# Sudaraka88/LDWeaver

Measured on AMD Instinct MI355X. Metric: MI SNP-pairs/sec, higher is better.
Workload: dtype i8

## Files before the change

include/ldweaver_amd_debug.h:

```cpp
#ifndef LDWEAVER_AMD_DEBUG_H
#define LDWEAVER_AMD_DEBUG_H

#include "ldweaver_amd.h"

#ifdef __cplusplus
extern "C" {
#endif

#define LDW_ENGINE_MFMA 0
#define LDW_ENGINE_HIST 1
#define LDW_ENGINE_HIST_STATES 2

int ldw_build_info(void);
int ldw_ctx_last_timing(ldw_ctx *ctx, double ms_out[4]);
int ldw_ctx_counters(ldw_ctx *ctx, int64_t out[4]);
int ldw_ctx_counters2(ldw_ctx *ctx, int64_t out[8]);
int ldw_gemm_stats(ldw_ctx *ctx, double out[6], int reset);
int ldw_apx_info(ldw_ctx *ctx, double out[6]);

int ldw_hamming_stats(ldw_ctx *ctx, double out[8]);
int ldw_joint_tables(ldw_ctx *ctx, const int32_t *pair_a, const int32_t *pair_b, int64_t npairs,
                     int64_t *counts_out, int64_t *fixed_out, int *frac_bits_out);

int ldw_set_engine(ldw_ctx *ctx, int engine);
int ldw_set_overlap(ldw_ctx *ctx, int on);
int ldw_set_fused(ldw_ctx *ctx, int on);
int ldw_set_mixed(ldw_ctx *ctx, int on);
int ldw_set_path(ldw_ctx *ctx, int mode);
int ldw_set_select(ldw_ctx *ctx, int mode);
int ldw_set_screen(ldw_ctx *ctx, int mode);
int ldw_set_prune(ldw_ctx *ctx, int on);
int ldw_set_pair_cap(uint32_t cap);
int ldw_reset_speculation(ldw_ctx *ctx);

int ldw_path_report(ldw_ctx *ctx, int64_t out[8], char *gate, int capacity);
int ldw_pair_form_report(ldw_ctx *ctx, int64_t out[5]);
int ldw_prune_report(ldw_ctx *ctx, int64_t out[4]);
int ldw_span_report(ldw_ctx *ctx, int64_t out[4]);
int ldw_overflow_report(ldw_ctx *ctx, int64_t out[4]);

int ldw_snp_bounds(ldw_ctx *ctx, double *out, int64_t capacity);
int ldw_debug_violations(ldw_ctx *ctx, double *out);
int ldw_debug_tab11(ldw_ctx *ctx, double W, double lo, double delta, double eta, double sprime, int32_t *out, double *cbin_out);
int ldw_debug_apx_params(ldw_ctx *ctx, double out[20], int64_t *vfixed_out, int64_t *vapx_out, int64_t capacity);
int ldw_debug_rows(ldw_ctx *ctx, int32_t *row0_out, uint32_t *slot_meta_out, int64_t capacity);
int ldw_debug_apx_gemm(ldw_ctx *ctx, const int32_t *rows_t, int nrt, const int32_t *rows_f, int nrf, int32_t *out);
int ldw_debug_screen_bound(ldw_ctx *ctx, int kind, int na, int nb, int64_t n, const int64_t *g, const int64_t *pa, const int64_t *pb, const float *pX, const float *pY,
                           const double *rr, const uint32_t *masks, const double params[20], float *out, double *out64);

int ldw_debug_plot_panels(ldw_ctx *ctx, const double *x, const double *y, const double *srp, const uint8_t *layer, const uint8_t *panel, int64_t n,
                          int on_device, const ldw_plot_opts *opts, int n_panels, int32_t W, int32_t H, uint8_t *rgb_out, double *stats_out,
                          int64_t *scratch_bytes_out, double *ms_out);
int ldw_debug_plot_colours(int kind, const double *t, int64_t n, uint8_t *rgb_out);
int ldw_tsv_stats(ldw_ctx *ctx, double *out10);
int ldw_tsv_set_variant(ldw_ctx *ctx, int variant);

#ifdef __cplusplus
}
#endif
#endif
```

ldweaver_amd/_lib.py:

```python
from __future__ import annotations

import ctypes as C
import os

import numpy as np

_HERE = os.path.dirname(os.path.abspath(__file__))
LIB_PATH = os.environ.get("LDW_AMD_LIB") or os.path.join(_HERE, "libldweaver_amd.so")

LDW_OK = 0
LDW_ERR_ARG, LDW_ERR_HIP, LDW_ERR_STATE, LDW_ERR_NOGPU, LDW_ERR_SIZE = 1, 2, 3, 4, 5
QUIRK_REFERENCE, QUIRK_INTENDED = 0, 1
MI_SR_ROWS_STAY = 1
ENGINE_MFMA, ENGINE_HIST, ENGINE_HIST_STATES = 0, 1, 2
COL_INT32, COL_INT64, COL_DOUBLE, COL_STR = 0, 1, 2, 3


class LdwError(RuntimeError):
    def __init__(self, code: int, msg: str):
        super().__init__(f"libldweaver_amd error {code}: {msg}")
        self.code = code


PLOT_SR_CLUST, PLOT_SR_COMBI, PLOT_LR, PLOT_LDMAP = 0, 1, 2, 3
# ... 99 lines not shown
    "ldw_write_alignment": (C.c_int, [_p, C.c_char_p, C.c_int, C.c_int, _p, _i64, C.c_char_p, _i64, _i64, C.POINTER(_i64)]),
    "ldw_write_table_tsv_str": (C.c_int, [C.c_char_p, C.c_int, _i64, C.c_int, _p, _p, _p, _p, _p, _i64, C.c_int, C.POINTER(_i64)]),
    "ldw_annot_snps": (C.c_int, [_p, _p, _i64, _p, _i64, _p, _i64, _p, _p, _i64, _p]),
    "ldw_annot_map": (C.c_int, [_p, _p, _p, _i64, _p, _i64, _p, C.POINTER(_i64), C.POINTER(_i64)]),
    "ldw_annot_links": (C.c_int, [_p, _p, _p, _i64, _p, _p, _i64, _i64, _p, _p, _p, _p, _p, C.POINTER(_i64)]),
    "ldw_plot_layout_get": (C.c_int, [C.c_int, C.c_int, C.c_double, C.c_double, C.c_double, C.c_double, _p]),
    "ldw_plot_ticks": (C.c_int, [C.c_double, C.c_double, C.c_int, C.c_int, _p, _p, _p, _p]),
    "ldw_png_write": (C.c_int, [C.c_char_p, _p, C.c_int32, C.c_int32, C.c_int, C.POINTER(_i64)]),
    "ldw_plot_scatter": (C.c_int, [_p, _p, _p, _p, _p, _p, _i64, C.c_int, _p, C.c_int, _p, C.c_char_p, _p, C.POINTER(_i64)]),
    "ldw_plot_links": (C.c_int, [_p, C.c_int, C.c_int, _p, C.c_char_p, _p, C.POINTER(_i64)]),
    "ldw_plot_heatmap": (C.c_int, [_p, _p, C.c_int32, C.c_int, C.c_char_p, C.c_char_p, _p]),
    "ldw_plot_ldmap": (C.c_int, [_p, C.c_int32, C.c_int32, C.c_int32, C.c_char_p, C.c_char_p, _p, _p, _p, _p, _i64]),
    "ldw_tsv_probe": (C.c_int, [C.c_char_p, C.c_int, C.POINTER(C.c_int32), C.POINTER(C.c_int32)]),
    "ldw_tsv_read": (C.c_int, [_p, C.c_char_p, C.c_int, C.c_int32, _i64, C.POINTER(_i64), C.POINTER(_i64), C.POINTER(C.c_uint32)]),
    "ldw_tsv_columns": (C.c_int, [_p, C.POINTER(_p), C.POINTER(_i64), C.POINTER(C.c_int32), C.POINTER(_i64)]),
    "ldw_tsv_fetch": (C.c_int, [_p, C.c_int32, _p, _i64, C.c_int]),
    "ldw_set_positions": (C.c_int, [_p, _p, _i64, C.c_double]),
    "ldw_links_load": (C.c_int, [_p, C.c_int, C.c_int32, C.c_int32, C.c_int32, C.c_int32, C.c_double, C.c_int32, C.POINTER(_i64)]),
    "ldw_compare_to_row": (C.c_int, [_p, _i64, _i64, _p, _i64, _p]),
    "ldw_vec_pos_match": (C.c_int, [_p, _i64, _p, _i64, _p]),
    "ldw_compare_triplet": (C.c_int, [_p, _p, _i64, C.c_double, C.POINTER(C.c_int)]),
    "ldw_fast_intersect": (C.c_int, [_p, _i64, _p, _i64, _p, C.POINTER(_i64)]),
}
_SIGS_DEBUG = {
    "ldw_build_info": (C.c_int, []),
    "ldw_ctx_last_timing": (C.c_int, [_p, _p]),
    "ldw_ctx_counters": (C.c_int, [_p, _p]),
    "ldw_ctx_counters2": (C.c_int, [_p, _p]),
    "ldw_gemm_stats": (C.c_int, [_p, _p, C.c_int]),
    "ldw_apx_info": (C.c_int, [_p, _p]),
    "ldw_hamming_stats": (C.c_int, [_p, _p]),
    "ldw_joint_tables": (C.c_int, [_p, _p, _p, _i64, _p, _p, _p]),
    "ldw_set_engine": (C.c_int, [_p, C.c_int]),
    "ldw_set_overlap": (C.c_int, [_p, C.c_int]),
    "ldw_set_fused": (C.c_int, [_p, C.c_int]),
    "ldw_set_mixed": (C.c_int, [_p, C.c_int]),
    "ldw_set_path": (C.c_int, [_p, C.c_int]),
    "ldw_set_select": (C.c_int, [_p, C.c_int]),
    "ldw_set_screen": (C.c_int, [_p, C.c_int]),
    "ldw_set_prune": (C.c_int, [_p, C.c_int]),
    "ldw_set_pair_cap": (C.c_int, [C.c_uint32]),
    "ldw_reset_speculation": (C.c_int, [_p]),
    "ldw_path_report": (C.c_int, [_p, _p, C.c_char_p, C.c_int]),
    "ldw_pair_form_report": (C.c_int, [_p, _p]),
    "ldw_prune_report": (C.c_int, [_p, _p]),
    "ldw_span_report": (C.c_int, [_p, _p]),
    "ldw_overflow_report": (C.c_int, [_p, _p]),
    "ldw_snp_bounds": (C.c_int, [_p, _p, C.c_int64]),
    "ldw_debug_violations": (C.c_int, [_p, _p]),
    "ldw_debug_tab11": (C.c_int, [_p, C.c_double, C.c_double, C.c_double, C.c_double, C.c_double, _p, _p]),
    "ldw_debug_apx_params": (C.c_int, [_p, _p, _p, _p, _i64]),
    "ldw_debug_rows": (C.c_int, [_p, _p, _p, _i64]),
    "ldw_debug_apx_gemm": (C.c_int, [_p, _p, C.c_int, _p, C.c_int, _p]),
    "ldw_debug_screen_bound": (C.c_int, [_p, C.c_int, C.c_int, C.c_int, _i64, _p, _p, _p, _p, _p, _p, _p, _p, _p, _p]),
    "ldw_debug_plot_panels": (C.c_int, [_p, _p, _p, _p, _p, _p, _i64, C.c_int, _p, C.c_int, C.c_int32, C.c_int32, _p, _p, C.POINTER(_i64), _p]),
    "ldw_debug_plot_colours": (C.c_int, [C.c_int, _p, _i64, _p]),
    "ldw_tsv_stats": (C.c_int, [_p, _p]),
    "ldw_tsv_set_variant": (C.c_int, [_p, C.c_int]),
}
_SIGS = {**_SIGS_API, **_SIGS_DEBUG}
_SIGS_BY_HEADER = {"ldweaver_amd.h": _SIGS_API, "ldweaver_amd_debug.h": _SIGS_DEBUG}


def declared_symbols(header: str | None = None):
    return sorted(_SIGS if header is None else _SIGS_BY_HEADER[header])


def lib():
    global _lib
    if _lib is None:
        if not os.path.exists(LIB_PATH):
            raise FileNotFoundError(
                f"{LIB_PATH} not found: build it with `make -C ldweaver_amd/csrc` or "
                "`python -c 'import __graft_entry__ as g; g.build()'` — there is no CPU fallback")
        try:
            import torch
        except ImportError:
            pass
        l = C.CDLL(LIB_PATH)
        for name, (res, args) in _SIGS.items():
            fn = getattr(l, name)
            fn.restype = res
            fn.argtypes = args
        _lib = l
    return _lib


def has_experiments() -> bool:
    return bool(lib().ldw_build_info() & 1)


def check(code: int):
    if code != LDW_OK:
        raise LdwError(code, lib().ldw_last_error().decode("utf-8", "replace"))


def ptr(a):
    if a is None:
        return None
    if isinstance(a, int):
        return C.c_void_p(a)
    if isinstance(a, np.ndarray):
        return C.c_void_p(a.ctypes.data)
    if hasattr(a, "data_ptr"):
        return C.c_void_p(a.data_ptr())
    raise TypeError(f"cannot take a pointer of {type(a)}")
# ... 6 lines not shown
```

ldweaver_amd/csrc/ldw_api.hip:

```cpp
#include <algorithm>
#include <atomic>
#include <chrono>
#include <cmath>
#include <cstdarg>
#include <cstdio>
#include <cstdlib>
#include <cstring>

#include <thread>
#include "ldw_internal.h"
#include "ldw_dev.h"
#include "ldw_fasta.h"
#include "ldw_links_read.h"

namespace ldw {
static thread_local char g_err[1024] = "";

void set_error(const char *fmt, ...) {
    va_list ap;
    va_start(ap, fmt);
    vsnprintf(g_err, sizeof(g_err), fmt, ap);
    va_end(ap);
}

// ... 384 lines not shown

int launch_fasta_count_pack(const uint8_t *chunk, int64_t rows, int64_t L, int64_t Lp, int32_t *counts, uint8_t *packed, hipStream_t s) {
    const int64_t lanes = (L + FA_COLS - 1) / FA_COLS;
    hipLaunchKernelGGL(k_fasta_count_pack, dim3((unsigned)((lanes + 255) / 256)), dim3(256), 0, s, chunk, rows, L, Lp, counts, packed);
    LDW_HIP(hipGetLastError());
    return LDW_OK;
}

int launch_fasta_encode_rows(bool packed, const uint8_t *src, int64_t stride, int64_t src_s0, int64_t s0, int64_t s_end, int64_t N,
                             const int32_t *pos, int64_t n_pos, uint8_t *states, int64_t Npad, hipStream_t s) {
    const dim3 grid((unsigned)((n_pos + 63) / 64), (unsigned)((s_end - s0 + 63) / 64));
    if (packed)
        hipLaunchKernelGGL(k_fasta_encode_rows<true>, grid, dim3(256), 0, s, src, stride, src_s0, s0, s_end, N, pos, n_pos, states, Npad);
    else
        hipLaunchKernelGGL(k_fasta_encode_rows<false>, grid, dim3(256), 0, s, src, stride, src_s0, s0, s_end, N, pos, n_pos, states, Npad);
    LDW_HIP(hipGetLastError());
    return LDW_OK;
}

}

extern "C" {

int ldw_version(void) { return 100; }

const char *ldw_last_error(void) { return ldw::g_err; }

int ldw_build_info(void) { return 0; }

int ldw_device_count(void) {
    int n = 0;
    if (hipGetDeviceCount(&n) != hipSuccess) return 0;
    return n;
}

int ldw_ctx_create(int device, ldw_ctx **out) {
    LDW_REQUIRE(out != nullptr, LDW_ERR_ARG, "ldw_ctx_create: out is null");
    int n = 0;
    if (hipGetDeviceCount(&n) != hipSuccess || n <= 0) {
        set_error("ldw_ctx_create: no HIP device visible; this library has no CPU fallback");
        return LDW_ERR_NOGPU;
    }
    LDW_REQUIRE(device >= 0 && device < n, LDW_ERR_ARG, "ldw_ctx_create: device %d out of range (0..%d)", device, n - 1);
    LDW_HIP(hipSetDevice(device));
    hipDeviceProp_t prop;
    LDW_HIP(hipGetDeviceProperties(&prop, device));
    if (strncmp(prop.gcnArchName, "gfx950", 6) != 0) {
        set_error("ldw_ctx_create: device %d is %s; kernels are built for gfx950 only", device, prop.gcnArchName);
        return LDW_ERR_NOGPU;
    }
    ldw_ctx *c = new ldw_ctx();
    ldw::ctx_count(+1);
    c->device = device;
    c->prune = getenv("LDW_NO_PRUNE") == nullptr;
    LDW_HIP(hipStreamCreateWithFlags(&c->stream, hipStreamNonBlocking));
    c->own_stream = true;
    for (auto &e : c->ev) LDW_HIP(hipEventCreate(&e));
    static const bool no_prep = getenv("LDW_NO_PREPARE") != nullptr;
    if (!no_prep) {
        if (int rc = ldw::ensure_streams(c)) {
            const std::string msg = ldw_last_error();
            ldw_ctx_destroy(c);
            *out = nullptr;
            ldw::set_error("%s", msg.c_str());
            return rc;
        }
        c->prep_thread = new std::thread([c] {
            int rc = LDW_OK;
            if (hipSetDevice(c->device) != hipSuccess) rc = LDW_ERR_HIP;
            if (rc == LDW_OK) {
                ldw::warm_mi();
                ldw::warm_apx();
                ldw::warm_gemm_bits();
                ldw::warm_srp();
                ldw::warm_post();
            }
            if (rc != LDW_OK) c->prep_err = ldw_last_error();
            c->prep_rc = rc;
        });
    }
    *out = c;
    return LDW_OK;
}

int ldw_ctx_reserve(ldw_ctx *c, int64_t L, int64_t N, int64_t max_blk_sz) {
    if (int rc = check_gpu(c)) return rc;
    LDW_REQUIRE(L > 0 && N > 0 && max_blk_sz > 0, LDW_ERR_ARG, "ldw_ctx_reserve: L, N and max_blk_sz must be positive");
    if (c->prep_thread2) {
        if (c->prep_thread2->joinable()) c->prep_thread2->join();
        delete c->prep_thread2;
        c->prep_thread2 = nullptr;
    }
    static const bool no_prep = getenv("LDW_NO_PREPARE") != nullptr;
    if (no_prep) return LDW_OK;
    const int64_t blk = std::min<int64_t>(L, max_blk_sz);
    const int64_t nblk = (L + blk - 1) / blk;
    const int64_t nseg = std::max<int64_t>(1, std::min<int64_t>(c->span_on ? c->span_max : 1, nblk - 2));
    const int64_t nt = blk * nseg, rows_f = blk * 5 / 4 + 512, rows_t = nt * 5 / 4 + 512;
    const size_t stage = (size_t)((blk + nt) * 12 + (rows_f + rows_t) * 9 + nt * 52 + (blk + 64) * 16 + 3 * (rows_t / 128 + 1) * (rows_f / 64 + 1) + 65536);
    const int64_t Npad = (N + ldw::KSTEP - 1) / ldw::KSTEP * ldw::KSTEP;
    c->prep_thread2 = new std::thread([c, stage, Npad, blk, nseg] {
        int rc = LDW_OK;
        if (hipSetDevice(c->device) != hipSuccess) rc = LDW_ERR_HIP;
        if (rc == LDW_OK) rc = ldw::reserve_slot_buffers(c, Npad, blk, nseg);
        for (int k = 0; k < LDW_NSLOT && rc == LDW_OK; ++k) {
            if (c->pin_cap[k] >= stage) continue;
// ... 767 lines not shown
```

ldweaver_amd/csrc/ldw_apx.hip:

```cpp
#include <algorithm>
#include <cmath>
#include <cstdlib>
#include <cstring>

#include "ldw_apx.h"
#include "ldw_dev.h"

using namespace ldw;

namespace ldw {

namespace {
constexpr int64_t APX_PROD_CAP = 12000;
struct ProdTable {
    std::vector<int32_t> val;
    std::vector<uint8_t> a, b;
    ProdTable() {
        std::vector<std::pair<int32_t, std::pair<uint8_t, uint8_t>>> all;
        for (int x = 0; x <= 127; ++x)
            for (int y = x; y <= 127; ++y) all.push_back({x * y, {(uint8_t)x, (uint8_t)y}});
        std::sort(all.begin(), all.end());
        for (auto &e : all)
            if (val.empty() || val.back() != e.first) {
                val.push_back(e.first);
// ... 321 lines not shown
        if (valid && !(P.sr_mask && P.sr_mask[(int64_t)((ty * TH) / 128) * (P.RFpad / 64) + tx] != 0)) {
            const TileSummary F = apx_fold_rows(P.bin_f + (int64_t)tx * TWd, P.rflag_f ? P.rflag_f + (int64_t)tx * TWd : nullptr, TWd);
            all_binned = T.bmax < P.tab_nb && F.bmax < P.tab_nb;
            if (P.rflag_t) {
                const unsigned kt = T.fand & PF_KIND, kf = F.fand & PF_KIND;
                pruned = kt >= 2u && kt == (T.forr & PF_KIND) && kf >= 2u && kf == (F.forr & PF_KIND) &&
                         ((T.fand & (kf == 2u ? PF_DEAD2 : PF_DEAD3)) != 0u || (F.fand & (kt == 2u ? PF_DEAD2 : PF_DEAD3)) != 0u);
            }
            if (!pruned && all_binned && (T.bmax - T.bmin + 1) * (F.bmax - F.bmin + 1) <= 64) {
                bool ok = true;
                for (int bt = T.bmin; bt <= T.bmax; ++bt)
                    for (int bf = F.bmin; bf <= F.bmax; ++bf) {
                        const int2 th = P.tab[bt * P.tab_nb + bf];
                        ok = ok && th.x < 0 && th.y == 2147483647;
                    }
                pruned = ok;
            }
        }
        if (pruned && all_binned) {
#pragma unroll
            for (int i = 0; i < MT; ++i)
#pragma unroll
                for (int h = 0; h < (NT * 32) / 64; ++h) P.clean[(int64_t)((ty * TH + 32 * i) / 32) * (P.RFpad / 64) + (tx * TWd) / 64 + h] = 1;
        }
        const bool live = valid && !pruned;
        const unsigned long long lm = __ballot(live);
        n_pruned += (unsigned int)__popcll(__ballot(valid && pruned));
        if (lane == 0) s_wave[wave] = (unsigned int)__popcll(lm);
        __syncthreads();
        if (threadIdx.x == 0) {
            const unsigned int tot = s_wave[0] + s_wave[1] + s_wave[2] + s_wave[3];
            s_base = tot ? atomicAdd(P.n_live, tot) : 0u;
        }
        __syncthreads();
        unsigned int off = s_base;
        for (int w = 0; w < wave; ++w) off += s_wave[w];
        if (live) P.tile_list[off + (unsigned int)__popcll(lm & ((1ull << lane) - 1ull))] = (uint32_t)(ty * ntx + tx);
        __syncthreads();
    }
    if (lane == 0 && n_pruned) atomicAdd(P.skip_ctr, (unsigned long long)n_pruned);
}

template <int MT, int NT, bool FINE, int WPS = 2>
__global__ __launch_bounds__(256, WPS) void gemm_apx_kernel(ApxGemmArgs P) {
    extern __shared__ __attribute__((aligned(16))) uint8_t smem[];
    uint64_t *lutFF = reinterpret_cast<uint64_t *>(smem);
    uint8_t *sA = smem + APX_LUT_BYTES, *sB = sA + (size_t)P.M2 * 128;
    int2 *s_tab = reinterpret_cast<int2 *>(sB + (size_t)P.M2 * 128);
    const int tid = threadIdx.x;
    const int lane = tid & 63, wave = tid >> 6;
    constexpr int TH = 32 * MT, TWd = 32 * NT;
    int ty = 2 * blockIdx.y + (wave >> 1), tx = 2 * blockIdx.x + (wave & 1);
    bool outside;
    if (P.tile_list) {
        const unsigned int n_live = *P.n_live;
        if (blockIdx.x * 4u >= n_live) return;
        const unsigned int k = blockIdx.x * 4u + (unsigned int)wave;
        outside = k >= n_live;
        const int t = outside ? 0 : (int)P.tile_list[k];
        const int ntx = P.RFpad / TWd;
        ty = t / ntx;
        tx = t - ty * ntx;
    } else {
        outside = ty * TH >= P.RTpad || tx * TWd >= P.RFpad || (P.lower_only && tx * TWd + TWd - 1 < ty * TH);
    }
    if (P.fuse)
        for (int i = tid; i < P.tab_nb * P.tab_nb; i += 256) s_tab[i] = P.tab[i];
    {
        uint64_t e = 0;
#pragma unroll
        for (int k = 0; k < 8; ++k) e |= ((tid >> k) & 1) ? (0xFFull << (8 * k)) : 0ull;
        lutFF[tid] = e;
        const int n16 = P.M2 * 8;
        for (int i = tid; i < n16; i += 256) {
            reinterpret_cast<uint4 *>(sA)[i] = reinterpret_cast<const uint4 *>(P.dig_a)[i];
            reinterpret_cast<uint4 *>(sB)[i] = reinterpret_cast<const uint4 *>(P.dig_b)[i];
        }
    }
    __syncthreads();
    if (outside) return;
    const int frow = lane & 31, fh = lane >> 5;
    const int64_t sta = (int64_t)P.RTpad * 2, stb = (int64_t)P.RFpad * 2;
    {
        const apx_u32x4 *pa[MT], *pb[NT];
#pragma unroll
        for (int i = 0; i < MT; ++i) {
            const int rt = ty * TH + 32 * i + frow;
            pa[i] = reinterpret_cast<const apx_u32x4 *>(P.panel_t) + ((int64_t)rt * 2 + fh);
        }
#pragma unroll
        for (int i = 0; i < NT; ++i) {
            const int rf = tx * TWd + 32 * i + frow;
            pb[i] = reinterpret_cast<const apx_u32x4 *>(P.panel_f) + ((int64_t)rf * 2 + fh);
        }
        v16i acc[MT][NT];
#pragma unroll
        for (int i = 0; i < MT; ++i)
#pragma unroll
            for (int j = 0; j < NT; ++j)
#pragma unroll
                for (int e = 0; e < 16; ++e) acc[i][j][e] = 0;
        apx_u32x4 wa[MT], wb[NT], na[MT], nb[NT];
        const uint8_t *lut_bytes = smem;
#pragma unroll
        for (int i = 0; i < MT; ++i) na[i] = pa[i][0];
#pragma unroll
        for (int i = 0; i < NT; ++i) nb[i] = pb[i][0];
        for (int m = 0; m < P.M2; ++m) {
#pragma unroll
            for (int i = 0; i < MT; ++i) wa[i] = na[i];
#pragma unroll
            for (int i = 0; i < NT; ++i) wb[i] = nb[i];
            if (m + 1 < P.M2) {
#pragma unroll
                for (int i = 0; i < MT; ++i) na[i] = pa[i][(int64_t)(m + 1) * sta];
#pragma unroll
                for (int i = 0; i < NT; ++i) nb[i] = pb[i][(int64_t)(m + 1) * stb];
            }
            const int4 sh4 = reinterpret_cast<const int4 *>(P.shift)[m];
            const int shk[4] = {sh4.x, sh4.y, sh4.z, sh4.w};
            const uint8_t *dA = sA + m * 128 + fh * (FINE ? 16 : 64), *dB = sB + m * 128 + fh * (FINE ? 16 : 64);
            auto kstep = [&](auto KKc) {
                constexpr int kk = decltype(KKc)::value;
                const int sh = shk[kk];
                if ((FINE || kk == 0) && sh) {
#pragma unroll
                    for (int i = 0; i < MT; ++i)
#pragma unroll
                        for (int j = 0; j < NT; ++j)
#pragma unroll
                            for (int e = 0; e < 16; ++e) acc[i][j][e] = (int)((unsigned)acc[i][j][e] >> sh);
                }
                const v4i da = *reinterpret_cast<const v4i *>(dA + (FINE ? 32 : 16) * kk);
                const v4i db = *reinterpret_cast<const v4i *>(dB + (FINE ? 32 : 16) * kk);
                v4i fa[MT], fb[NT];
#pragma unroll
                for (int i = 0; i < MT; ++i) fa[i] = expand16s<kk>(lut_bytes, wa[i]) & da;
#pragma unroll
                for (int i = 0; i < NT; ++i) fb[i] = expand16s<kk>(lut_bytes, wb[i]) & db;
#pragma unroll
                for (int i = 0; i < MT; ++i)
#pragma unroll
                    for (int j = 0; j < NT; ++j) acc[i][j] = __builtin_amdgcn_mfma_i32_32x32x32_i8(fa[i], fb[j], acc[i][j], 0, 0, 0);
            };
            kstep(std::integral_constant<int, 0>{});
            kstep(std::integral_constant<int, 1>{});
            kstep(std::integral_constant<int, 2>{});
            kstep(std::integral_constant<int, 3>{});
        }
        apx_gemm_epilogue<MT, NT>(P, acc, ty, tx, lane, s_tab, reinterpret_cast<uint8_t *>(s_tab + 64 * 64) + wave * 256);
    }
}

int launch_apx_live_tiles(ldw_ctx *c, const ApxGemmArgs &P, hipStream_t st) {
    LDW_REQUIRE(P.fuse && P.skip_ctr && P.tile_list && P.n_live && P.RTpad % 128 == 0 && P.RFpad % 64 == 0 && P.tab && P.tab_nb == 64,
                LDW_ERR_ARG, "launch_apx_live_tiles: bad pruning arguments");
    hipLaunchKernelGGL(k_apx_live_tiles, dim3((unsigned)(P.RTpad / (32 * APX_MT))), dim3(256), 0, st, P);
    LDW_HIP(hipGetLastError());
    return LDW_OK;
}

int launch_gemm_apx(ldw_ctx *c, const ApxGemmArgs &P, hipStream_t st) {
    LDW_REQUIRE(P.RTpad % APX_TW == 0 && P.RFpad % APX_TW == 0 && P.M2 > 0, LDW_ERR_ARG, "launch_gemm_apx: padding violated (RT %d RF %d M2 %d)", P.RTpad,
                P.RFpad, P.M2);
    const size_t lds = APX_LUT_BYTES + (size_t)P.M2 * 256 + (P.fuse ? (size_t)P.tab_nb * P.tab_nb * 8 + 1024 : 0);
    LDW_REQUIRE(lds <= 65536, LDW_ERR_ARG, "launch_gemm_apx: %d positions do not fit the LDS digit arrays", P.M2 * 128);
    LDW_REQUIRE(!P.fuse || (P.tab_nb == 64 && P.bin_t && P.bin_f && P.tab && P.clean), LDW_ERR_ARG, "launch_gemm_apx: bad table arguments");
    if (P.skip_ctr) {
        LDW_REQUIRE(P.fuse && P.tile_list && P.n_live && P.RFpad % 64 == 0, LDW_ERR_ARG, "launch_gemm_apx: bad pruning arguments");
        const int tiles = (P.RTpad / (32 * APX_MT)) * (P.RFpad / 64), g = (tiles + 3) / 4;
        if (P.fine) hipLaunchKernelGGL((gemm_apx_kernel<APX_MT, 2, true, APX_WPS>), dim3((unsigned)g), dim3(256), lds, st, P);
        else hipLaunchKernelGGL((gemm_apx_kernel<APX_MT, 2, false, APX_WPS>), dim3((unsigned)g), dim3(256), lds, st, P);
    } else {
        const int ntx = P.RFpad / 64, nty = P.RTpad / 128;
        const dim3 grid((unsigned)((ntx + 1) / 2), (unsigned)((nty + 1) / 2));
        if (P.fine) hipLaunchKernelGGL((gemm_apx_kernel<4, 2, true>), grid, dim3(256), lds, st, P);
        else hipLaunchKernelGGL((gemm_apx_kernel<4, 2, false>), grid, dim3(256), lds, st, P);
    }
    LDW_HIP(hipGetLastError());
    {
        constexpr int TH = 128, TWd = 64;
        int64_t waves = 0;
        for (int ty = 0; ty * TH < P.RTpad; ++ty) {
            const int ntx = P.RFpad / TWd;
            if (!P.lower_only) waves += ntx;
            else for (int tx = 0; tx < ntx; ++tx) waves += (tx * TWd + TWd - 1 < ty * TH) ? 0 : 1;
        }
        c->gemm_stat[0] += 1;
        if (P.fuse) c->gemm_stat[5] += 1;
        c->gemm_stat[1] += 2.0 * (double)waves * TH * TWd * ((double)P.M2 * 128.0);
        if (P.fuse && P.skip_ctr) {
            c->apx_ops_per_wave = 2.0 * TH * TWd * ((double)P.M2 * 128.0);
            c->apx_waves_total += waves;
        }
    }
    return LDW_OK;
}

struct PairArgs {
    const uint64_t *Mbits;
    int64_t KW;
    int nwords, path, nseg;
    int seg_in_lds;
    const PopSeg *segs;
    const int32_t *wbeg, *row0;
    int32_t zero_row;
    int64_t *sums;
    EpiArgs A;
    unsigned long long *ghist;
};

template <int CA, int CB>
__device__ __forceinline__ void pair_sums_body(const PairArgs &P, int path, const int32_t *s_wbeg, const PopSeg *s_segs) {
    constexpr bool GENB = CA == 4 && CB == 4;
    const EpiArgs &A = P.A;
    const int sub = path * PAIR_SHARDS + (int)blockIdx.y;
    unsigned int n = A.pl_n[sub];
    n = n > A.pl_cap ? A.pl_cap : n;
    const int lane = threadIdx.x & 63;
    const PairEnt *list = A.pl_pairs + (int64_t)sub * A.pl_cap;
    constexpr int KW = 3, KS = 2;
    uint32_t smask[KW][KS];
    int64_t sV[KW][KS];
// ... 363 lines not shown
```

ldweaver_amd/csrc/ldw_debug.hip:

```cpp
#include <algorithm>
#include <cmath>
#include <cstring>
#include <vector>

#include "ldw_apx.h"
#include "ldw_dev.h"

using namespace ldw;

namespace ldw {

struct DbgArrays {
    const int64_t *g;
    const int32_t *g32;
    const int64_t *pa, *pb;
    const float *pX, *pY;
    const double *rr;
    const uint32_t *mk;
    float *out;
    double *out64;
    int64_t n;
};

template <int NA, int NB>
// ... 118 lines not shown
    if (int rc = check_gpu(c)) return rc;
    if (int rc = ensure_rows(c)) return rc;
    LDW_REQUIRE(row0_out && slot_meta_out && capacity >= c->L + 1, LDW_ERR_ARG, "ldw_debug_rows: need L + 1 = %lld entries", (long long)c->L + 1);
    memcpy(row0_out, c->h_row0.data(), (size_t)(c->L + 1) * 4);
    memcpy(slot_meta_out, c->h_slot_meta.data(), (size_t)c->L * 4);
    return LDW_OK;
}

int ldw_debug_apx_gemm(ldw_ctx *c, const int32_t *rows_t, int nrt, const int32_t *rows_f, int nrf, int32_t *out) {
    if (int rc = check_gpu(c)) return rc;
    if (int rc = join_prepare(c)) return rc;
    if (int rc = ensure_rows(c)) return rc;
    LDW_REQUIRE(rows_t && rows_f && out && nrt > 0 && nrf > 0 && nrt <= 8192 && nrf <= 8192, LDW_ERR_ARG, "ldw_debug_apx_gemm: bad argument");
    LDW_REQUIRE(c->apx_ok, LDW_ERR_STATE, "ldw_debug_apx_gemm: the weights do not allow the approximate path (%s)", c->apx_gate.c_str());
    for (int k = 0; k < nrt; ++k) LDW_REQUIRE(rows_t[k] >= 0 && rows_t[k] <= c->R, LDW_ERR_ARG, "ldw_debug_apx_gemm: to-side row %d = %d outside 0..R", k, rows_t[k]);
    for (int k = 0; k < nrf; ++k) LDW_REQUIRE(rows_f[k] >= 0 && rows_f[k] <= c->R, LDW_ERR_ARG, "ldw_debug_apx_gemm: from-side row %d = %d outside 0..R", k, rows_f[k]);
    const int RTpad = (nrt + APX_TW - 1) / APX_TW * APX_TW, RFpad = (nrf + APX_TW - 1) / APX_TW * APX_TW, M2 = (int)(c->KW / 2);
    std::vector<int32_t> rl((size_t)RTpad + RFpad, (int32_t)c->R);
    std::copy(rows_t, rows_t + nrt, rl.begin());
    std::copy(rows_f, rows_f + nrf, rl.begin() + RTpad);
    DevBuf d_rl, d_pt, d_pf, d_G;
    int rc = LDW_OK;
    if ((rc = d_rl.reserve(rl.size() * 4)) || (rc = d_pt.reserve((size_t)M2 * RTpad * 32)) || (rc = d_pf.reserve((size_t)M2 * RFpad * 32)) ||
        (rc = d_G.reserve((size_t)RTpad * RFpad * 4))) {
        d_rl.release(); d_pt.release(); d_pf.release(); d_G.release();
        return rc;
    }
    auto body = [&]() -> int {
        LDW_HIP(hipMemcpyAsync(d_rl.p, rl.data(), rl.size() * 4, hipMemcpyHostToDevice, c->stream));
        LDW_HIP(hipMemsetAsync(d_G.p, 0xFF, (size_t)RTpad * RFpad * 4, c->stream));
        if (int r2 = launch_pack_panel(c, d_rl.as<int32_t>() + RTpad, RFpad, d_pf.as<uint64_t>(), c->stream, d_rl.as<int32_t>(), RTpad, d_pt.as<uint64_t>())) return r2;
        ApxGemmArgs P;
        memset(&P, 0, sizeof(P));
        P.panel_t = d_pt.as<uint64_t>();
        P.panel_f = d_pf.as<uint64_t>();
        P.RTpad = RTpad;
        P.RFpad = RFpad;
        P.M2 = M2;
        P.dig_a = c->dig_a.as<uint8_t>();
        P.dig_b = c->dig_b.as<uint8_t>();
        P.shift = c->apx_shift.as<int32_t>();
        P.G = d_G.as<int32_t>();
        P.fine = c->apx_fine ? 1 : 0;
        if (int r2 = launch_gemm_apx(c, P, c->stream)) return r2;
        std::vector<int32_t> h((size_t)RTpad * RFpad);
        LDW_HIP(hipMemcpyAsync(h.data(), d_G.p, h.size() * 4, hipMemcpyDeviceToHost, c->stream));
        LDW_HIP(hipStreamSynchronize(c->stream));
        for (int t = 0; t < nrt; ++t) memcpy(out + (size_t)t * nrf, h.data() + (size_t)t * RFpad, (size_t)nrf * 4);
        return LDW_OK;
    };
    rc = body();
    (void)hipStreamSynchronize(c->stream);
    d_rl.release(); d_pt.release(); d_pf.release(); d_G.release();
    return rc;
}

int ldw_debug_screen_bound(ldw_ctx *c, int kind, int na, int nb, int64_t n, const int64_t *g, const int64_t *pa, const int64_t *pb, const float *pX, const float *pY,
                           const double *rr, const uint32_t *masks, const double params[20], float *out, double *out64) {
    if (int rc = check_gpu(c)) return rc;
    LDW_REQUIRE(n > 0 && n < ((int64_t)1 << 28) && g && pa && pb && pX && pY && rr && params, LDW_ERR_ARG, "ldw_debug_screen_bound: bad argument");
    LDW_REQUIRE(kind >= 0 && kind <= 4 && ((kind == 4) ? out64 != nullptr : out != nullptr), LDW_ERR_ARG, "ldw_debug_screen_bound: kind %d / missing output", kind);
    const bool generic = kind == 1 || kind == 3;
    LDW_REQUIRE(generic ? masks != nullptr : ((na == 1 || na == 2) && (nb == 1 || nb == 2)), LDW_ERR_ARG, "ldw_debug_screen_bound: kinds 0 / 2 / 4 take na, nb in {1, 2}; kinds 1 / 3 take masks");
    const bool apx = kind == 0 || kind == 1;
    std::vector<int32_t> g32;
    if (apx) {
        g32.resize((size_t)n * 16);
        for (size_t k = 0; k < g32.size(); ++k) {
            LDW_REQUIRE(g[k] >= -2147483647LL && g[k] <= 2147483647LL, LDW_ERR_ARG, "ldw_debug_screen_bound: entry %zu does not fit int32", k);
            g32[k] = (int32_t)g[k];
        }
    }
    DevBuf B;
    const size_t sz_g = (size_t)n * 16 * 8, sz_g32 = (size_t)n * 16 * 4, sz_p = (size_t)n * 5 * 8, sz_f = (size_t)n * 5 * 4, sz_r = (size_t)n * 3 * 8, sz_m = (size_t)n * 2 * 4,
                 sz_o = (size_t)n * 4, sz_o64 = (size_t)n * 8;
    auto al = [](size_t x) { return (x + 255) / 256 * 256; };
    const size_t o_g = 0, o_g32 = o_g + al(sz_g), o_pa = o_g32 + al(sz_g32), o_pb = o_pa + al(sz_p), o_pX = o_pb + al(sz_p), o_pY = o_pX + al(sz_f), o_rr = o_pY + al(sz_f),
                 o_m = o_rr + al(sz_r), o_o = o_m + al(sz_m), o_o64 = o_o + al(sz_o), total = o_o64 + al(sz_o64);
    if (int rc = B.reserve(total)) return rc;
    char *base = B.as<char>();
    auto body = [&]() -> int {
        LDW_HIP(hipMemcpyAsync(base + o_g, g, sz_g, hipMemcpyHostToDevice, c->stream));
        if (apx) LDW_HIP(hipMemcpyAsync(base + o_g32, g32.data(), sz_g32, hipMemcpyHostToDevice, c->stream));
        LDW_HIP(hipMemcpyAsync(base + o_pa, pa, sz_p, hipMemcpyHostToDevice, c->stream));
        LDW_HIP(hipMemcpyAsync(base + o_pb, pb, sz_p, hipMemcpyHostToDevice, c->stream));
        LDW_HIP(hipMemcpyAsync(base + o_pX, pX, sz_f, hipMemcpyHostToDevice, c->stream));
        LDW_HIP(hipMemcpyAsync(base + o_pY, pY, sz_f, hipMemcpyHostToDevice, c->stream));
        LDW_HIP(hipMemcpyAsync(base + o_rr, rr, sz_r, hipMemcpyHostToDevice, c->stream));
        if (masks) LDW_HIP(hipMemcpyAsync(base + o_m, masks, sz_m, hipMemcpyHostToDevice, c->stream));
        EpiArgs A;
        memset(&A, 0, sizeof(A));
        A.neff = params[5];
        A.scale = std::ldexp(1.0, -(int)params[0]);
        A.quirk = LDW_QUIRK_INTENDED;
        A.E.apx = apx ? 1 : 0;
        A.E.apx_EG = (float)params[6];
        A.E.apx_dfac = (float)params[7];
        A.E.apx_s1 = (float)params[8];
        A.E.apx_c1 = (float)params[9];
        A.E.apx_W = params[10];
        A.E.apx_unit = params[11];
        A.E.apx_MU = (float)params[18];
        A.E.scr_shift = apx ? 0 : (int)params[13];
        A.E.scr_scale = (float)(apx ? params[12] : params[14]);
        DbgArrays D;
        D.g = reinterpret_cast<const int64_t *>(base + o_g);
// ... 38 lines not shown
```

ldweaver_amd/csrc/ldw_internal.h:

```cpp
#pragma once
#include <hip/hip_runtime.h>
#include <stdint.h>
#include <stdlib.h>
#include <string>
#include <atomic>
#include <memory>
#include <mutex>
#include <thread>
#include <vector>

#include "../../include/ldweaver_amd.h"
#include "../../include/ldweaver_amd_debug.h"

#define LDW_NSLOT 3


namespace ldw {

void set_error(const char *fmt, ...);
int hip_fail(hipError_t e, const char *what, const char *file, int line);

#define LDW_HIP(call)                                                        \
    do {                                                                     \
        hipError_t e__ = (call);                                             \
        if (e__ != hipSuccess) return ldw::hip_fail(e__, #call, __FILE__, __LINE__); \
    } while (0)

#define LDW_REQUIRE(cond, code, ...)   \
    do {                               \
        if (!(cond)) {                 \
            ldw::set_error(__VA_ARGS__); \
            return (code);             \
        }                              \
    } while (0)

struct DevBuf {
    void *p = nullptr;
    size_t cap = 0;
    int reserve(size_t bytes);
    int reserve_keep(size_t bytes, size_t used, hipStream_t s);
    void release();
    template <class T> T *as() const { return reinterpret_cast<T *>(p); }
};

constexpr int TILE = 128;
constexpr int KSTEP = 128;
constexpr int NBINS = 4096;

struct BlockStat {
    int64_t n_lr_total = 0, n_lr_kept = 0, n_sr = 0;
    double disc_thresh = 0;
};
struct BlockTrace {
    int diag = 0, guess = -1, B_true = -1, margin = 0, path = 0 , missed = 0, probed = 0;
    long long n_cand = 0;
};

}

struct ldw_ctx {
    int device = 0;
    hipStream_t stream = nullptr;
    bool own_stream = true;
    hipEvent_t ev[6] = {nullptr, nullptr, nullptr, nullptr, nullptr, nullptr};
    double last_ms[4] = {0, 0, 0, 0};
    int engine = LDW_ENGINE_MFMA;

    int64_t L = 0, N = 0, Npad = 0;
    int64_t KW = 0;
    ldw::DevBuf states;
    ldw::DevBuf chars;
    int64_t cN = 0, cL = 0;
    void *fasta = nullptr;
    void *out = nullptr;
    void *tsv = nullptr;

    bool have_weights = false;
    int nlimbs = 5;
    int frac_bits = 0;
    double neff = 0;
    int64_t total_fixed = 0;
    ldw::DevBuf digits;
    ldw::DevBuf vfixed;
    std::vector<int64_t> h_vfixed;
    std::vector<int64_t> h_vfixed_hi;
    int64_t total_fixed_hi = 0;
    double lo_abs_sum = 0;
    int mixed = 1;

    std::vector<int32_t> h_seq_perm;
    ldw::DevBuf seq_perm;
    int path_mode = 0;
    int select_mode = 0;
    bool apx_ok = false;
    bool apx_fine = false;
    std::string apx_gate = "weights not set";
    ldw::DevBuf dig_a, dig_b;
    ldw::DevBuf apx_shift;
    int apx_e_last = 0;
    int apx_transitions = 0;
    double apx_lost_units = 0;
    double apx_delta = 0;
    std::vector<int64_t> h_vapx;
    ldw::DevBuf slot_papx;
    ldw::DevBuf pop_segs, pop_wbeg;
    ldw::DevBuf pop_vpos;
    bool pair_bits_attr = false;
    int n_pop_segs = 0, n_classes = 0;
    ldw::DevBuf panel[LDW_NSLOT][2];
    ldw::DevBuf Gapx[LDW_NSLOT];
    ldw::DevBuf tab11[2];
    double tab11_lo[2] = {0, 0};
    int tab11_cur[2] = {0, 0};
    int64_t tab11_builds = 0;
// ... 177 lines not shown
```

ldweaver_amd/engine.py:

```python
from __future__ import annotations

import ctypes as C
import errno
import os

import numpy as np

from . import _lib as L

ANNOT_REC = 12


def fasta_check(code: int, path):
    if code == L.LDW_OK:
        return
    msg = L.lib().ldw_last_error().decode("utf-8", "replace")
    if "does not contain any sequences" in msg:
        raise ValueError("File does not contain any sequences!")
    if "sequences are of different lengths" in msg:
        raise ValueError("Error! sequences are of different lengths!")
    if "cannot open" in msg:
        raise FileNotFoundError(errno.ENOENT, msg, str(path)) if not os.path.exists(path) else OSError(msg)
    raise L.LdwError(code, msg)

# ... 92 lines not shown
            n_rows = int(n.value)
        dev = torch.device("cuda", self.device)
        a = torch.empty(max(1, n_rows), dtype=torch.int32, device=dev)
        b = torch.empty(max(1, n_rows), dtype=torch.int32, device=dev)
        torch.cuda.synchronize(dev)
        L.check(L.lib().ldw_sr_pairs_fill(self._ctx, L.ptr(bl), len(bl), float(sr_dist), C.c_void_p(a.data_ptr()), C.c_void_p(b.data_ptr()), n_rows, C.byref(n)))
        assert int(n.value) == n_rows, (int(n.value), n_rows)
        return a[:n_rows], b[:n_rows]

    def set_span(self, on: bool, max_blocks: int = 0, corners: bool = False, diag_split: bool = False):
        L.check(L.lib().ldw_set_span(self._ctx, (1 if on else 0) | (2 if (on and corners) else 0) | (4 if (on and diag_split) else 0), int(max_blocks)))

    def span_report(self):
        v = np.zeros(4, dtype=np.int64)
        L.check(L.lib().ldw_span_report(self._ctx, L.ptr(v)))
        return dict(spans=int(v[0]), blocks=int(v[1]), redone=int(v[2]), on=bool(v[3]))

    def overflow_report(self):
        v = np.zeros(4, dtype=np.int64)
        L.check(L.lib().ldw_overflow_report(self._ctx, L.ptr(v)))
        return dict(pair_list=int(v[0]), maybe_list=int(v[1]), maybe_off=bool(v[2]), maybe_entries=int(v[3]))

    @staticmethod
    def set_pair_cap(cap: int):
        L.check(L.lib().ldw_set_pair_cap(int(cap)))

    def snp_bounds(self):
        out = np.zeros(4 * self.L)
        L.check(L.lib().ldw_snp_bounds(self._ctx, L.ptr(out), out.size))
        return out.reshape(self.L, 2, 2)

    APX_PARAM_NAMES = ("F", "e_last", "delta", "lost_units", "total_fixed", "neff", "apx_EG", "apx_dfac", "apx_s1", "apx_c1", "apx_W", "apx_unit", "scr_scale",
                       "scr_shift_exact", "scr_scale_exact", "flags", "lo_abs_sum", "lo_bound", "apx_MU", "nlimbs")

    def debug_apx_params(self, want_weights: bool = True):
        out = np.zeros(20)
        V = np.zeros(self.N if want_weights else 0, dtype=np.int64)
        Va = np.zeros(self.N if want_weights else 0, dtype=np.int64)
        L.check(L.lib().ldw_debug_apx_params(self._ctx, L.ptr(out), L.ptr(V) if want_weights else None, L.ptr(Va) if want_weights else None, self.N))
        return out, V, Va

    def debug_rows(self):
        row0 = np.zeros(self.L + 1, dtype=np.int32)
        meta = np.zeros(self.L, dtype=np.uint32)
        L.check(L.lib().ldw_debug_rows(self._ctx, L.ptr(row0), L.ptr(meta), self.L + 1))
        return row0, meta

    def debug_apx_gemm(self, rows_t, rows_f):
        rt = np.ascontiguousarray(rows_t, dtype=np.int32)
        rf = np.ascontiguousarray(rows_f, dtype=np.int32)
        out = np.zeros((len(rt), len(rf)), dtype=np.int32)
        L.check(L.lib().ldw_debug_apx_gemm(self._ctx, L.ptr(rt), len(rt), L.ptr(rf), len(rf), L.ptr(out)))
        return out

    def debug_screen_bound(self, kind: int, na: int, nb: int, g, pa, pb, pX, pY, rr, params, masks=None):
        g = np.ascontiguousarray(g, dtype=np.int64).reshape(-1, 16)
        n = len(g)
        pa = np.ascontiguousarray(pa, dtype=np.int64).reshape(n, 5)
        pb = np.ascontiguousarray(pb, dtype=np.int64).reshape(n, 5)
        pX = np.ascontiguousarray(pX, dtype=np.float32).reshape(n, 5)
        pY = np.ascontiguousarray(pY, dtype=np.float32).reshape(n, 5)
        rr = np.ascontiguousarray(rr, dtype=np.float64).reshape(n, 3)
        params = np.ascontiguousarray(params, dtype=np.float64).reshape(20)
        mk = None if masks is None else np.ascontiguousarray(masks, dtype=np.uint32).reshape(n, 2)
        out = np.zeros(n, dtype=np.float32)
        out64 = np.zeros(n, dtype=np.float64)
        L.check(L.lib().ldw_debug_screen_bound(self._ctx, int(kind), int(na), int(nb), n, L.ptr(g), L.ptr(pa), L.ptr(pb), L.ptr(pX), L.ptr(pY), L.ptr(rr),
                                               L.ptr(mk), L.ptr(params), L.ptr(out), L.ptr(out64)))
        return out64 if kind == 4 else out

    def write_links_tsv(self, which: int, path: str, append: bool = True, nthreads: int = 0):
        n, nb = C.c_int64(0), C.c_int64(0)
        L.check(L.lib().ldw_write_links_tsv(self._ctx, int(which), str(path).encode(), int(bool(append)), int(nthreads), C.byref(n), C.byref(nb)))
        return int(n.value), int(nb.value)

    def host_trim(self) -> int:
        n = C.c_int64(0)
        L.check(L.lib().ldw_host_trim(self._ctx, C.byref(n)))
        return int(n.value)

    def lr_stream_begin(self, path: str, append: bool = True, nthreads: int = 0):
        L.check(L.lib().ldw_lr_stream_begin(self._ctx, str(path).encode(), int(bool(append)), int(nthreads)))

    def lr_stream_end(self):
        n, nb, blk = C.c_int64(0), C.c_int64(0), C.c_int64(0)
        L.check(L.lib().ldw_lr_stream_end(self._ctx, C.byref(n), C.byref(nb), C.byref(blk)))
        return int(n.value), int(nb.value), int(blk.value)

    def write_links_tsv_begin(self, which: int, path: str, append: bool = True, nthreads: int = 0):
        L.check(L.lib().ldw_write_links_tsv_begin(self._ctx, int(which), str(path).encode(), int(bool(append)), int(nthreads)))

    def write_links_tsv_end(self):
        n, nb = C.c_int64(0), C.c_int64(0)
        L.check(L.lib().ldw_write_links_tsv_end(self._ctx, C.byref(n), C.byref(nb)))
        return int(n.value), int(nb.value)

    def set_overlap(self, on: bool):
        L.check(L.lib().ldw_set_overlap(self._ctx, int(bool(on))))

    def set_fused(self, on: bool):
        L.check(L.lib().ldw_set_fused(self._ctx, int(bool(on))))

    def set_mixed(self, on: bool):
        L.check(L.lib().ldw_set_mixed(self._ctx, int(bool(on))))

    def set_path(self, mode: int):
# ... 616 lines not shown
```

Baseline: 169.3 billion.

## Make pruned APX GEMM kernel persistent over live tile list, cap grid to CUs

```diff
diff --git a/include/ldweaver_amd_debug.h b/include/ldweaver_amd_debug.h
--- a/include/ldweaver_amd_debug.h
+++ b/include/ldweaver_amd_debug.h
@@ -45,6 +45,8 @@
 int ldw_debug_apx_params(ldw_ctx *ctx, double out[20], int64_t *vfixed_out, int64_t *vapx_out, int64_t capacity);
 int ldw_debug_rows(ldw_ctx *ctx, int32_t *row0_out, uint32_t *slot_meta_out, int64_t capacity);
 int ldw_debug_apx_gemm(ldw_ctx *ctx, const int32_t *rows_t, int nrt, const int32_t *rows_f, int nrf, int32_t *out);
+int ldw_debug_apx_tiles(ldw_ctx *ctx, const int32_t *rows_t, int nrt, const int32_t *rows_f, int nrf, const uint8_t *bin_t, const uint8_t *bin_f, const int32_t *tab,
+                        int lower_only, int maybe_cap, int32_t *g_out, uint8_t *clean_out, int32_t *maybe_out, int64_t counts[4]);
 int ldw_debug_screen_bound(ldw_ctx *ctx, int kind, int na, int nb, int64_t n, const int64_t *g, const int64_t *pa, const int64_t *pb, const float *pX, const float *pY,
                            const double *rr, const uint32_t *masks, const double params[20], float *out, double *out64);
 
diff --git a/ldweaver_amd/_lib.py b/ldweaver_amd/_lib.py
--- a/ldweaver_amd/_lib.py
+++ b/ldweaver_amd/_lib.py
@@ -175,6 +175,7 @@
     "ldw_debug_apx_params": (C.c_int, [_p, _p, _p, _p, _i64]),
     "ldw_debug_rows": (C.c_int, [_p, _p, _p, _i64]),
     "ldw_debug_apx_gemm": (C.c_int, [_p, _p, C.c_int, _p, C.c_int, _p]),
+    "ldw_debug_apx_tiles": (C.c_int, [_p, _p, C.c_int, _p, C.c_int, _p, _p, _p, C.c_int, C.c_int, _p, _p, _p, _p]),
     "ldw_debug_screen_bound": (C.c_int, [_p, C.c_int, C.c_int, C.c_int, _i64, _p, _p, _p, _p, _p, _p, _p, _p, _p, _p]),
     "ldw_debug_plot_panels": (C.c_int, [_p, _p, _p, _p, _p, _p, _i64, C.c_int, _p, C.c_int, C.c_int32, C.c_int32, _p, _p, C.POINTER(_i64), _p]),
     "ldw_debug_plot_colours": (C.c_int, [C.c_int, _p, _i64, _p]),
diff --git a/ldweaver_amd/csrc/ldw_api.hip b/ldweaver_amd/csrc/ldw_api.hip
--- a/ldweaver_amd/csrc/ldw_api.hip
+++ b/ldweaver_amd/csrc/ldw_api.hip
@@ -460,6 +460,7 @@
     ldw_ctx *c = new ldw_ctx();
     ldw::ctx_count(+1);
     c->device = device;
+    c->n_cu = prop.multiProcessorCount;
     c->prune = getenv("LDW_NO_PRUNE") == nullptr;
     LDW_HIP(hipStreamCreateWithFlags(&c->stream, hipStreamNonBlocking));
     c->own_stream = true;
diff --git a/ldweaver_amd/csrc/ldw_apx.hip b/ldweaver_amd/csrc/ldw_apx.hip
--- a/ldweaver_amd/csrc/ldw_apx.hip
+++ b/ldweaver_amd/csrc/ldw_apx.hip
@@ -397,36 +397,59 @@
     constexpr int TH = 32 * MT, TWd = 32 * NT;
     int ty = 2 * blockIdx.y + (wave >> 1), tx = 2 * blockIdx.x + (wave & 1);
     bool outside;
+    unsigned int n_live = 0, k = 0;
+    const unsigned int kstride = 4u * gridDim.x;
     if (P.tile_list) {
-        const unsigned int n_live = *P.n_live;
+        n_live = *P.n_live;
         if (blockIdx.x * 4u >= n_live) return;
-        const unsigned int k = blockIdx.x * 4u + (unsigned int)wave;
+        k = (unsigned int)__builtin_amdgcn_readfirstlane((int)(blockIdx.x * 4u + (unsigned int)wave));
         outside = k >= n_live;
-        const int t = outside ? 0 : (int)P.tile_list[k];
-        const int ntx = P.RFpad / TWd;
-        ty = t / ntx;
-        tx = t - ty * ntx;
     } else {
         outside = ty * TH >= P.RTpad || tx * TWd >= P.RFpad || (P.lower_only && tx * TWd + TWd - 1 < ty * TH);
     }
-    if (P.fuse)
-        for (int i = tid; i < P.tab_nb * P.tab_nb; i += 256) s_tab[i] = P.tab[i];
     {
         uint64_t e = 0;
 #pragma unroll
-        for (int k = 0; k < 8; ++k) e |= ((tid >> k) & 1) ? (0xFFull << (8 * k)) : 0ull;
+        for (int b = 0; b < 8; ++b) e |= ((tid >> b) & 1) ? (0xFFull << (8 * b)) : 0ull;
         lutFF[tid] = e;
         const int n16 = P.M2 * 8;
-        for (int i = tid; i < n16; i += 256) {
-            reinterpret_cast<uint4 *>(sA)[i] = reinterpret_cast<const uint4 *>(P.dig_a)[i];
-            reinterpret_cast<uint4 *>(sB)[i] = reinterpret_cast<const uint4 *>(P.dig_b)[i];
-        }
+        for (int i0 = tid; i0 < n16; i0 += 1024) {
+            uint4 qa[4], qb[4];
+#pragma unroll
+            for (int q = 0; q < 4; ++q) {
+                const int i = min(i0 + 256 * q, n16 - 1);
+                qa[q] = reinterpret_cast<const uint4 *>(P.dig_a)[i];
+                qb[q] = reinterpret_cast<const uint4 *>(P.dig_b)[i];
+            }
+#pragma unroll
+            for (int q = 0; q < 4; ++q) {
+                const int i = i0 + 256 * q;
+                if (i < n16) {
+                    reinterpret_cast<uint4 *>(sA)[i] = qa[q];
+                    reinterpret_cast<uint4 *>(sB)[i] = qb[q];
+                }
+            }
+        }
+    }
+    if (P.fuse) {
+        uint4 tq[8];
+#pragma unroll
+        for (int q = 0; q < 8; ++q) tq[q] = reinterpret_cast<const uint4 *>(P.tab)[tid + 256 * q];
+#pragma unroll
+        for (int q = 0; q < 8; ++q) reinterpret_cast<uint4 *>(s_tab)[tid + 256 * q] = tq[q];
     }
     __syncthreads();
     if (outside) return;
-    const int frow = lane & 31, fh = lane >> 5;
     const int64_t sta = (int64_t)P.RTpad * 2, stb = (int64_t)P.RFpad * 2;
-    {
+    for (;;) {
+        int ln = lane;
+        if (P.tile_list) {
+            const int t = __builtin_amdgcn_readfirstlane((int)P.tile_list[k]), ntx = P.RFpad / TWd;
+            ty = t / ntx;
+            tx = t - ty * ntx;
+            ln |= t >> 31;
+        }
+        const int frow = lane & 31, fh = lane >> 5;
         const apx_u32x4 *pa[MT], *pb[NT];
 #pragma unroll
         for (int i = 0; i < MT; ++i) {
@@ -493,7 +516,10 @@
             kstep(std::integral_constant<int, 2>{});
             kstep(std::integral_constant<int, 3>{});
         }
-        apx_gemm_epilogue<MT, NT>(P, acc, ty, tx, lane, s_tab, reinterpret_cast<uint8_t *>(s_tab + 64 * 64) + wave * 256);
+        apx_gemm_epilogue<MT, NT>(P, acc, ty, tx, ln, s_tab, reinterpret_cast<uint8_t *>(s_tab + 64 * 64) + wave * 256);
+        if (!P.tile_list) break;
+        k += kstride;
+        if (k >= n_live) break;
     }
 }
 
@@ -513,7 +539,13 @@
     LDW_REQUIRE(!P.fuse || (P.tab_nb == 64 && P.bin_t && P.bin_f && P.tab && P.clean), LDW_ERR_ARG, "launch_gemm_apx: bad table arguments");
     if (P.skip_ctr) {
         LDW_REQUIRE(P.fuse && P.tile_list && P.n_live && P.RFpad % 64 == 0, LDW_ERR_ARG, "launch_gemm_apx: bad pruning arguments");
-        const int tiles = (P.RTpad / (32 * APX_MT)) * (P.RFpad / 64), g = (tiles + 3) / 4;
+        const int tiles = (P.RTpad / (32 * APX_MT)) * (P.RFpad / 64), g_all = (tiles + 3) / 4;
+        int g_max = 2 * (c->n_cu > 0 ? c->n_cu : 256);
+        if (const char *e = getenv("LDW_APX_GRID")) {
+            const int v = atoi(e);
+            g_max = v > 0 ? v : (v == 0 ? g_all : g_max);
+        }
+        const int g = std::min(g_all, g_max);
         if (P.fine) hipLaunchKernelGGL((gemm_apx_kernel<APX_MT, 2, true, APX_WPS>), dim3((unsigned)g), dim3(256), lds, st, P);
         else hipLaunchKernelGGL((gemm_apx_kernel<APX_MT, 2, false, APX_WPS>), dim3((unsigned)g), dim3(256), lds, st, P);
     } else {
diff --git a/ldweaver_amd/csrc/ldw_debug.hip b/ldweaver_amd/csrc/ldw_debug.hip
--- a/ldweaver_amd/csrc/ldw_debug.hip
+++ b/ldweaver_amd/csrc/ldw_debug.hip
@@ -194,6 +194,94 @@
     rc = body();
     (void)hipStreamSynchronize(c->stream);
     d_rl.release(); d_pt.release(); d_pf.release(); d_G.release();
+    return rc;
+}
+
+int ldw_debug_apx_tiles(ldw_ctx *c, const int32_t *rows_t, int nrt, const int32_t *rows_f, int nrf, const uint8_t *bin_t, const uint8_t *bin_f, const int32_t *tab,
+                        int lower_only, int maybe_cap, int32_t *g_out, uint8_t *clean_out, int32_t *maybe_out, int64_t counts[4]) {
+    if (int rc = check_gpu(c)) return rc;
+    if (int rc = join_prepare(c)) return rc;
+    if (int rc = ensure_rows(c)) return rc;
+    LDW_REQUIRE(rows_t && rows_f && bin_t && bin_f && tab && g_out && clean_out && counts && nrt > 0 && nrf > 0 && nrt <= 8192 && nrf <= 8192 && nrt % APX_TW == 0 &&
+                    nrf % APX_TW == 0 && maybe_cap >= 0 && (maybe_cap == 0 || maybe_out),
+                LDW_ERR_ARG, "ldw_debug_apx_tiles: bad argument (row counts are multiples of %d: pad with row R)", APX_TW);
+    LDW_REQUIRE(c->apx_ok, LDW_ERR_STATE, "ldw_debug_apx_tiles: the weights do not allow the approximate path (%s)", c->apx_gate.c_str());
+    for (int k = 0; k < nrt; ++k) LDW_REQUIRE(rows_t[k] >= 0 && rows_t[k] <= c->R, LDW_ERR_ARG, "ldw_debug_apx_tiles: to-side row %d = %d outside 0..R", k, rows_t[k]);
+    for (int k = 0; k < nrf; ++k) LDW_REQUIRE(rows_f[k] >= 0 && rows_f[k] <= c->R, LDW_ERR_ARG, "ldw_debug_apx_tiles: from-side row %d = %d outside 0..R", k, rows_f[k]);
+    const int M2 = (int)(c->KW / 2);
+    const size_t n_tiles = (size_t)(nrt / 128) * (size_t)(nrf / 64), n_clean = (size_t)(nrt / 32) * (size_t)(nrf / 64);
+    auto al = [](size_t x) { return (x + 255) / 256 * 256; };
+    const size_t o_rl = 0, o_bt = o_rl + al(((size_t)nrt + nrf) * 4), o_bf = o_bt + al((size_t)nrt), o_tab = o_bf + al((size_t)nrf), o_cnt = o_tab + al(64 * 64 * 8),
+                 o_tl = o_cnt + 256, o_cl = o_tl + al(n_tiles * 4), o_mb = o_cl + al(n_clean), total = o_mb + al((size_t)maybe_cap * sizeof(ApxMaybe));
+    DevBuf d_w, d_pt, d_pf, d_G;
+    int rc = LDW_OK;
+    if ((rc = d_w.reserve(total)) || (rc = d_pt.reserve((size_t)M2 * nrt * 32)) || (rc = d_pf.reserve((size_t)M2 * nrf * 32)) || (rc = d_G.reserve((size_t)nrt * nrf * 4))) {
+        d_w.release(); d_pt.release(); d_pf.release(); d_G.release();
+        return rc;
+    }
+    const double st0 = c->gemm_stat[0], st1 = c->gemm_stat[1], st5 = c->gemm_stat[5], opw = c->apx_ops_per_wave;
+    const int64_t wt = c->apx_waves_total;
+    char *base = d_w.as<char>();
+    auto body = [&]() -> int {
+        LDW_HIP(hipMemsetAsync(base, 0, total, c->stream));
+        LDW_HIP(hipMemcpyAsync(base + o_rl, rows_t, (size_t)nrt * 4, hipMemcpyHostToDevice, c->stream));
+        LDW_HIP(hipMemcpyAsync(base + o_rl + (size_t)nrt * 4, rows_f, (size_t)nrf * 4, hipMemcpyHostToDevice, c->stream));
+        LDW_HIP(hipMemcpyAsync(base + o_bt, bin_t, (size_t)nrt, hipMemcpyHostToDevice, c->stream));
+        LDW_HIP(hipMemcpyAsync(base + o_bf, bin_f, (size_t)nrf, hipMemcpyHostToDevice, c->stream));
+        LDW_HIP(hipMemcpyAsync(base + o_tab, tab, 64 * 64 * 8, hipMemcpyHostToDevice, c->stream));
+        LDW_HIP(hipMemsetAsync(d_G.p, 0xFF, (size_t)nrt * nrf * 4, c->stream));
+        const int32_t *rl = reinterpret_cast<const int32_t *>(base + o_rl);
+        if (int r2 = launch_pack_panel(c, rl + nrt, nrf, d_pf.as<uint64_t>(), c->stream, rl, nrt, d_pt.as<uint64_t>())) return r2;
+        unsigned int *cnt = reinterpret_cast<unsigned int *>(base + o_cnt);
+        ApxGemmArgs P;
+        memset(&P, 0, sizeof(P));
+        P.panel_t = d_pt.as<uint64_t>();
+        P.panel_f = d_pf.as<uint64_t>();
+        P.RTpad = nrt;
+        P.RFpad = nrf;
+        P.M2 = M2;
+        P.dig_a = c->dig_a.as<uint8_t>();
+        P.dig_b = c->dig_b.as<uint8_t>();
+        P.shift = c->apx_shift.as<int32_t>();
+        P.G = d_G.as<int32_t>();
+        P.lower_only = lower_only ? 1 : 0;
+        P.fine = c->apx_fine ? 1 : 0;
+        P.fuse = 1;
+        P.bin_t = reinterpret_cast<const uint8_t *>(base + o_bt);
+        P.bin_f = reinterpret_cast<const uint8_t *>(base + o_bf);
+        P.tab = reinterpret_cast<const int2 *>(base + o_tab);
+        P.tab_nb = 64;
+        P.clean = reinterpret_cast<uint8_t *>(base + o_cl);
+        P.skip_ctr = reinterpret_cast<unsigned long long *>(cnt + 2);
+        P.tile_list = reinterpret_cast<uint32_t *>(base + o_tl);
+        P.n_live = cnt;
+        if (maybe_cap > 0) {
+            P.maybe = reinterpret_cast<ApxMaybe *>(base + o_mb);
+            P.maybe_n = cnt + 1;
+            P.maybe_cap = (unsigned int)maybe_cap;
+        }
+        if (int r2 = launch_apx_live_tiles(c, P, c->stream)) return r2;
+        if (int r2 = launch_gemm_apx(c, P, c->stream)) return r2;
+        unsigned int h_cnt[4];
+        LDW_HIP(hipMemcpyAsync(h_cnt, cnt, sizeof(h_cnt), hipMemcpyDeviceToHost, c->stream));
+        LDW_HIP(hipMemcpyAsync(g_out, d_G.p, (size_t)nrt * nrf * 4, hipMemcpyDeviceToHost, c->stream));
+        LDW_HIP(hipMemcpyAsync(clean_out, base + o_cl, n_clean, hipMemcpyDeviceToHost, c->stream));
+        if (maybe_cap > 0) LDW_HIP(hipMemcpyAsync(maybe_out, base + o_mb, (size_t)maybe_cap * sizeof(ApxMaybe), hipMemcpyDeviceToHost, c->stream));
+        LDW_HIP(hipStreamSynchronize(c->stream));
+        counts[0] = h_cnt[0];
+        counts[1] = h_cnt[1];
+        counts[2] = (int64_t)(((unsigned long long)h_cnt[3] << 32) | h_cnt[2]);
+        counts[3] = (int64_t)n_tiles;
+        return LDW_OK;
+    };
+    rc = body();
+    (void)hipStreamSynchronize(c->stream);
+    c->gemm_stat[0] = st0;
+    c->gemm_stat[1] = st1;
+    c->gemm_stat[5] = st5;
+    c->apx_ops_per_wave = opw;
+    c->apx_waves_total = wt;
+    d_w.release(); d_pt.release(); d_pf.release(); d_G.release();
     return rc;
 }
 
diff --git a/ldweaver_amd/csrc/ldw_internal.h b/ldweaver_amd/csrc/ldw_internal.h
--- a/ldweaver_amd/csrc/ldw_internal.h
+++ b/ldweaver_amd/csrc/ldw_internal.h
@@ -60,6 +60,7 @@
 
 struct ldw_ctx {
     int device = 0;
+    int n_cu = 0;
     hipStream_t stream = nullptr;
     bool own_stream = true;
     hipEvent_t ev[6] = {nullptr, nullptr, nullptr, nullptr, nullptr, nullptr};
diff --git a/ldweaver_amd/engine.py b/ldweaver_amd/engine.py
--- a/ldweaver_amd/engine.py
+++ b/ldweaver_amd/engine.py
@@ -168,6 +168,25 @@
         out = np.zeros((len(rt), len(rf)), dtype=np.int32)
         L.check(L.lib().ldw_debug_apx_gemm(self._ctx, L.ptr(rt), len(rt), L.ptr(rf), len(rf), L.ptr(out)))
         return out
+
+    def debug_apx_tiles(self, rows_t, rows_f, bin_t, bin_f, tab, lower_only: bool = False, maybe_cap: int = 0):
+        rt = np.ascontiguousarray(rows_t, dtype=np.int32)
+        rf = np.ascontiguousarray(rows_f, dtype=np.int32)
+        bt = np.ascontiguousarray(bin_t, dtype=np.uint8)
+        bf = np.ascontiguousarray(bin_f, dtype=np.uint8)
+        tb = np.ascontiguousarray(tab, dtype=np.int32)
+        assert len(bt) == len(rt) and len(bf) == len(rf) and tb.shape == (64, 64, 2)
+        G = np.zeros((len(rt), len(rf)), dtype=np.int32)
+        clean = np.zeros((len(rt) // 32, len(rf) // 64), dtype=np.uint8)
+        mb = np.zeros((max(maybe_cap, 1), 3), dtype=np.int32)
+        counts = np.zeros(4, dtype=np.int64)
+        L.check(L.lib().ldw_debug_apx_tiles(self._ctx, L.ptr(rt), len(rt), L.ptr(rf), len(rf), L.ptr(bt), L.ptr(bf), L.ptr(tb), int(bool(lower_only)), int(maybe_cap),
+                                            L.ptr(G), L.ptr(clean), L.ptr(mb) if maybe_cap > 0 else None, L.ptr(counts)))
+        n = int(min(counts[1], maybe_cap))
+        m = mb[:n].astype(np.int64)
+        m[:, :2] &= 0xFFFFFFFF
+        m = m[np.lexsort((m[:, 2], m[:, 1], m[:, 0]))]
+        return dict(G=G, clean=clean, maybe=m, maybe_n=int(counts[1]), n_live=int(counts[0]), n_pruned=int(counts[2]), n_tiles=int(counts[3]))
 
     def debug_screen_bound(self, kind: int, na: int, nb: int, g, pa, pb, pX, pY, rr, params, masks=None):
         g = np.ascontiguousarray(g, dtype=np.int64).reshape(-1, 16)
```

After: 155.4 billion. -8.2%, worse.
